# david-gimeno/tailored-avsr

Measured on AMD Instinct MI355X. Metric: utterances/sec fwd+bwd, 12L tailored AV-Branchformer (Conv3d+ResNet-18 lip frontend, fusion, CTC+6L decoder), 4 s clips, batch 32/GPU, higher is better.
Workload: dtype f32

## Files before the change

### tailored-avsr_amd/csrc/gemm.hip

```cpp
#include <algorithm>

#include <cstdlib>
#include "gemm_glds.h"

namespace tavsr {

template <int V>
__global__ __launch_bounds__(256) void splitk_epilogue_kernel(const GemmArgs args) {
  const tavsr_gemm_desc& d = args.d;
  const int64_t mn = (int64_t)d.M * d.N;
  const int nbatch = d.nb1 * d.nb2;
  const int64_t i = ((int64_t)blockIdx.x * 256 + threadIdx.x) * V;
  const int z = blockIdx.y, z1 = z / d.nb2, z2 = z % d.nb2;
  if (d.a_rowsum && z == 0 && i < d.M) {
    const float* rs = d.ws + (int64_t)args.nsplit * nbatch * mn;
    for (int q = 0; q < V && i + q < d.M; ++q) {
      float v = 0.f;
      for (int s = 0; s < args.nsplit; ++s) v += rs[(int64_t)s * d.M + i + q];
      d.a_rowsum[i + q] = d.alpha * v;
    }
  }
  if (i >= mn) return;
  const int m = (int)(i / d.N), n = (int)(i % d.N);
  float v[V];
// ... 154 lines not shown
    __syncthreads();
    int kt0 = 0;
    for (; kt0 + 2 * PF < nk; kt0 += PF) {
#pragma unroll
      for (int u = 0; u < PF; ++u) kstep(kt0 + u, ra[(u + 1) % PF], rb[(u + 1) % PF], true, true, fast_tag);
    }
    for (; kt0 < nk; kt0 += PF) {
#pragma unroll
      for (int u = 0; u < PF; ++u) {
        const int kt = kt0 + u;
        if (kt < nk) kstep(kt, ra[(u + 1) % PF], rb[(u + 1) % PF], kt + 1 < nk, kt + 1 + PF < nk, fast_tag);
      }
    }
  };
  if (fast) run_loop(std::true_type{});
  else run_loop(std::false_type{});

  finish_tile<TM, TN>(d, args.nsplit, acc, asum, want_rowsum, m0, n0, wm, wn, lr, lk, z1, z2, coff, (int)blockIdx.z);
}

__device__ float g_zero_page[16];

template <int ROWS, bool KMAJOR, int NT, bool B_SIDE>
struct TailOperand : PlainOperand<ROWS, KMAJOR, NT, B_SIDE> {
  using P = PlainOperand<ROWS, KMAJOR, NT, B_SIDE>;
  int kofs[P::L::NR];
  __device__ __forceinline__ explicit TailOperand(const TileCtx& c_) : P(c_) {
#pragma unroll
    for (int i = 0; i < P::L::NR; ++i) {
      const int q = i * NT + this->c.tid;
      kofs[i] = KMAJOR ? q / (ROWS / 4) : ((q & 7) ^ (((q >> 3) >> 1) & 7)) * 4;
    }
  }
  __device__ __forceinline__ void issue(int kt, float* img) {
    const TileCtx& c = this->c;
    const int kleft = c.kend - (c.kbeg + kt * kBK);
    const float* g = this->gk + kt * this->kstep;
#pragma unroll
    for (int i = 0; i < P::L::NR; ++i) {
      const float* chunk = g + this->off[i];
      dma16(kofs[i] < kleft ? chunk : g_zero_page, img + (i * NT + c.wave * 64) * 4);
    }
  }
  __device__ __forceinline__ static void zero_past(float* img, int kt_len, int tid) {
    const int k4 = (kt_len + 3) & ~3;
    if (!KMAJOR)
      for (int r = tid; r < ROWS; r += NT)
        for (int kk = kt_len; kk < k4; ++kk) img[r * 32 + ((((kk >> 2) ^ ((r >> 1) & 7))) << 2) + (kk & 3)] = 0.f;
  }
};

template <int BM, int BN, int NT, bool AK, bool BKM>
struct TailSource : SourceDefaults {
  using HA = TailOperand<BM, AK, NT, false>;
  using HB = TailOperand<BN, BKM, NT, true>;
  static constexpr int kDma = HA::kDma + HB::kDma;
  const TileCtx& c;
  HA a;
  HB b;
  __device__ __forceinline__ explicit TailSource(const TileCtx& c_) : c(c_), a(c_), b(c_) {}
  __device__ __forceinline__ int steps() const { return (c.kend - c.kbeg + kBK - 1) / kBK; }
  __device__ __forceinline__ void issue(int kt, float* stage) {
    a.issue(kt, stage);
    b.issue(kt, stage + BM * kBK);
  }
  __device__ __forceinline__ void fix_last(float* stage, int klen, int kt, int tid) const {
    const int kt_len = klen - kt * kBK;
    HA::zero_past(stage, kt_len, tid);
    HB::zero_past(stage + BM * kBK, kt_len, tid);
    __syncthreads();
  }
};
template <int BM, int BN, int NT, bool AK, bool BKM>
struct SourceFor<3, false, BM, BN, NT, AK, BKM> {
  using type = TailSource<BM, BN, NT, AK, BKM>;
};

constexpr int kMaxGroup = 12;
struct GroupArgs {
  tavsr_gemm_desc d[kMaxGroup];
  int tile_start[kMaxGroup + 1];
  int tiles_n[kMaxGroup];
  int n;
  int vec_epi;
};

template <int BM, int BN, int WM, int WN, int S, int MINW, bool AK, bool BKM>
__global__ __launch_bounds__(WM* WN * 64, MINW)
void gemm_glds_grouped_kernel(const GroupArgs g) {
  const int bid = xcd_remap(blockIdx.x, gridDim.x);
  int pi = 0;
#pragma unroll
  for (int i = 1; i < kMaxGroup; ++i)
    if (i < g.n && bid >= g.tile_start[i]) pi = i;
  glds_tile<BM, BN, WM, WN, S, AK, BKM>(g.d[pi], g.d[pi].K, 1, g.tiles_n[pi], bid - g.tile_start[pi], g.vec_epi != 0, 0);
}

// ... 438 lines not shown
```

### tailored-avsr_amd/csrc/gemm_conv.hip

```cpp
#include <algorithm>
#include <vector>

#include "gemm_glds.h"

namespace tavsr {

constexpr int kOrdRuns = 80;
struct TileOrder {
  int nruns;
  int start[kOrdRuns];
  int cum[kOrdRuns + 1];
  int w[kOrdRuns];
};

__host__ __device__ inline void tile_order_map(const TileOrder& o, int b, int tiles_m, int tiles_n, int& mt, int& nt) {
  const int per = 8 * tiles_n;
  const int g = b / per, j = b - g * per, s0 = 8 * g;
  int r0 = 0;
  while (r0 + 1 < o.nruns && o.cum[r0 + 1] <= s0) ++r0;
  bool uniform = s0 + 8 <= tiles_m;
  if (uniform) {
    int r7 = r0;
    while (r7 + 1 < o.nruns && o.cum[r7 + 1] <= s0 + 7) ++r7;
    uniform = o.w[r7] == o.w[r0];
// ... 12 lines not shown
  const unsigned long long taps = (H - 1) * W >= H * (W - 1) ? 0x862053714ull : 0x862071534ull;
  const int tap = (int)((taps >> (4 * rank)) & 15);
  return (rem / tpt) * tiles_n + tap * tpt + rem % tpt;
}

__host__ __device__ inline void dw_xcd_order(int j, int tiles_m, int tiles_n, int ns, int& zs, int& q) {
  const int tiles = tiles_m * tiles_n;
  zs = j / tiles;
  q = j - zs * tiles;
  if (tiles_n % 9 != 0) return;
  const int per = tiles_m * (tiles_n / 9);
  const int rank = j / (ns * per), rem = j - rank * (ns * per);
  zs = rem / per;
  q = rank * per + rem - zs * per;
}

struct ConvGeom {
  int cs, p0, Ho, Wo;
  bool c9;
  __device__ __forceinline__ explicit ConvGeom(const tavsr_gemm_desc& d) {
    cs = d.conv_stride > 1 ? d.conv_stride : 1;
    c9 = d.conv_taps != 1;
    p0 = d.conv_taps == 90 ? 1 : 0;
    Ho = (d.conv_H - 1 - 2 * p0) / cs + 1;
    Wo = (d.conv_W - 1 - 2 * p0) / cs + 1;
  }
};

template <int BM, int NT>
struct ImageRows {
  using L = GLoader<BM, false, NT>;
  int64_t off[L::NR];
  uint32_t mask[L::NR];
  __device__ __forceinline__ void issue(const TileCtx& c, bool c9, int kk, int tap, float* img) const {
    const tavsr_gemm_desc& d = c.d;
    const int toff = c9 ? (tap / 3 - 1) * d.conv_W + (tap % 3 - 1) : 0;
    const int64_t delta = (int64_t)toff * d.conv_C + (kk - tap * d.conv_C);
#pragma unroll
    for (int i = 0; i < L::NR; ++i)
      dma16(((mask[i] >> tap) & 1u) ? c.A + off[i] + delta : d.conv_zero, img + (i * NT + c.wave * 64) * 4);
  }
};

template <int BM, int NT>
struct ConvRowsA {
  using R = ImageRows<BM, NT>;
  static constexpr int kDma = R::L::NR;
  const TileCtx& c;
  bool c9;
  R rows;
  __device__ __forceinline__ explicit ConvRowsA(const TileCtx& c_) : c(c_) {
    const tavsr_gemm_desc& d = c.d;
    const ConvGeom g(d);
    c9 = g.c9;
    R::L::offsets(d.lda, c.m0, d.M, c.tid, rows.off);
#pragma unroll
    for (int i = 0; i < R::L::NR; ++i) {
      const int m = min(c.m0 + ((i * NT + c.tid) >> 3), d.M - 1);
      const int x = (m % g.Wo) * g.cs + g.p0, y = ((m / g.Wo) % g.Ho) * g.cs + g.p0;
      if (g.cs > 1 || g.p0) rows.off[i] += ((int64_t)((m / (g.Wo * g.Ho)) * d.conv_H + y) * d.conv_W + x - m) * d.conv_C;
      uint32_t mk = 0;
#pragma unroll
      for (int tap = 0; tap < 9; ++tap)
        mk |= (uint32_t)((unsigned)(y + tap / 3 - 1) < (unsigned)d.conv_H && (unsigned)(x + tap % 3 - 1) < (unsigned)d.conv_W) << tap;
      rows.mask[i] = g.c9 ? mk : 1u;
    }
  }
  __device__ __forceinline__ void issue(int kt, float* img) {
    const int kk = c.kbeg + kt * kBK;
    rows.issue(c, c9, kk, kk / c.d.conv_C, img);
  }
};
template <int BM, int BN, int NT, bool BKM>
struct SourceFor<1, false, BM, BN, NT, false, BKM> {
  using type = PairSource<ConvRowsA<BM, NT>, PlainOperand<BN, BKM, NT, true>, BM>;
};

template <int BM, int BN, int NT, bool BKM>
struct PosMajorRowsSource : SourceDefaults {
  using R = ImageRows<BM, NT>;
  using LB = GLoader<BN, BKM, NT>;
  static constexpr int kDma = R::L::NR + LB::NR;
  static constexpr bool kPosMajorRows = true;
  const TileCtx& c;
  PosMajor pm{};
  uint32_t taps = 0;
  int tap, cb, nk;
  bool c9;
  R rows;
  int64_t offB[LB::NR];
  __device__ __forceinline__ explicit PosMajorRowsSource(const TileCtx& c_) : c(c_) {
    const tavsr_gemm_desc& d = c.d;
    const ConvGeom g(d);
    c9 = g.c9;
    LB::offsets(d.ldb, c.n0, d.N, c.tid, offB);
    pm.H = g.Ho; pm.W = g.Wo;
    pm.st = g.cs; pm.HI = d.conv_H; pm.WI = d.conv_W;
    pm.n = d.M / (g.Ho * g.Wo);
    const int vlo = c.m0 / pm.n, vhi = min(c.m0 + BM - 1, d.M - 1) / pm.n;
    for (int v = vlo; v <= vhi; ++v) {
      int y, x;
      pm.pos(v, y, x);
      taps |= pm.taps(y, x);
      pm.rp = y * g.Wo + x;
    }
    pm.uni = vlo == vhi;
    pm.base = vlo * pm.n;
    nk = 0;
    for (int t = 0; t < 9; ++t) {
      const int lo = max(c.kbeg, t * d.conv_C), hi = min(c.kend, (t + 1) * d.conv_C);
      if (((taps >> t) & 1u) && hi > lo) nk += (hi - lo) / kBK;
    }
    tap = c.kbeg / d.conv_C;
    cb = (c.kbeg - tap * d.conv_C) / kBK;
    if (!((taps >> tap) & 1u)) {
      const uint32_t up = taps >> (tap + 1) << (tap + 1);
      tap = up ? __builtin_ctz(up) : 9;
      cb = 0;
    }
#pragma unroll
    for (int i = 0; i < R::L::NR; ++i) {
      const int q = i * NT + c.tid, row = q >> 3;
      const int r = min(c.m0 + row, d.M - 1);
      int y, x, img;
      if (pm.uni) {
        y = pm.rp / g.Wo; x = pm.rp - y * g.Wo; img = r - pm.base;
      } else {
        const int v = r / pm.n;
        pm.pos(v, y, x);
        img = r - v * pm.n;
      }
      rows.off[i] = ((int64_t)img * (d.conv_H * d.conv_W) + g.cs * y * d.conv_W + g.cs * x) * d.lda + ((q & 7) ^ ((row >> 1) & 7)) * 4;
      rows.mask[i] = pm.taps(y, x);
    }
  }
  __device__ __forceinline__ int steps() const { return nk; }
  __device__ __forceinline__ const PosMajor* row_map() const { return &pm; }
  __device__ __forceinline__ void issue(int, float* stage) {
    const tavsr_gemm_desc& d = c.d;
    const int ktap = tap, kk = tap * d.conv_C + cb * kBK;
    const int wrap = (cb + 1) * kBK >= d.conv_C;
    const uint32_t up = taps >> (tap + 1) << (tap + 1);
    cb = wrap ? 0 : cb + 1;
    tap = !wrap ? tap : up ? __builtin_ctz(up) : 9;
    rows.issue(c, c9, kk, ktap, stage);
    LB::issue(c.B + (BKM ? (int64_t)kk * d.ldb : kk), offB, stage + BM * kBK, c.wave);
  }
};
template <int BM, int BN, int NT, bool BKM>
struct SourceFor<1, true, BM, BN, NT, false, BKM> {
  using type = PosMajorRowsSource<BM, BN, NT, BKM>;
};

template <int BN, int NT>
struct PatchB {
  using L = GLoader<BN, true, NT>;
  static constexpr int kDma = L::NR;
  const TileCtx& c;
  const ConvGeom g;
  int ox[L::NR], oy[L::NR], img[L::NR];
  int sb, salo, sahi, tapoff, cb, dy, dx;
  __device__ __forceinline__ explicit PatchB(const TileCtx& c_) : c(c_), g(c_.d) {
    const tavsr_gemm_desc& d = c.d;
    const int sa = kBK / g.Wo;
    sb = kBK - sa * g.Wo;
    sahi = sa / g.Ho;
    salo = sa - sahi * g.Ho;
    const int tap = c.n0 / d.conv_C;
    cb = c.n0 - tap * d.conv_C;
    dy = g.c9 ? tap / 3 - 1 : 0;
    dx = g.c9 ? tap % 3 - 1 : 0;
    tapoff = dy * d.conv_W + dx;
#pragma unroll
    for (int i = 0; i < L::NR; ++i) {
      const int m = c.kbeg + (i * NT + c.tid) / (BN / 4);
      const int t = m / g.Wo;
      ox[i] = m - t * g.Wo;
      img[i] = t / g.Ho;
      oy[i] = t - img[i] * g.Ho;
    }
  }
  __device__ __forceinline__ void issue(int, float* dst) {
    const tavsr_gemm_desc& d = c.d;
#pragma unroll
    for (int i = 0; i < L::NR; ++i) {
      const int r = (((i * NT + c.tid) % (BN / 4)) * 4);
      const int x = ox[i] * g.cs + g.p0, y = oy[i] * g.cs + g.p0;
      const bool ok = (unsigned)(y + dy) < (unsigned)d.conv_H && (unsigned)(x + dx) < (unsigned)d.conv_W;
      const int64_t pix = (int64_t)(img[i] * d.conv_H + y) * d.conv_W + x;
      dma16(ok ? c.B + (pix + tapoff) * d.conv_C + cb + r : d.conv_zero, dst + (i * NT + c.wave * 64) * 4);
      int nx = ox[i] + sb;
      const int w1 = nx >= g.Wo ? 1 : 0;
      nx -= w1 ? g.Wo : 0;
      int ny = oy[i] + salo + w1;
      const int w2 = ny >= g.Ho ? 1 : 0;
      ny -= w2 ? g.Ho : 0;
      ox[i] = nx; oy[i] = ny; img[i] += sahi + w2;
    }
  }
};
template <int BM, int BN, int NT>
struct SourceFor<2, false, BM, BN, NT, true, true> {
  using type = PairSource<PlainOperand<BM, true, NT, false>, PatchB<BN, NT>, BM>;
};

template <int BM, int BN, int NT>
struct PatchWalkSource : SourceDefaults {
  using LA = GLoader<BM, true, NT>;
  using LB = GLoader<BN, true, NT>;
  static constexpr int kDma = LA::NR + LB::NR;
  const TileCtx& c;
  const ConvGeom g;
  int64_t offA[LA::NR];
  int tapoff, cb, dy, dx;
  int n, i0, nk;
  int v = 0, img = 0, x = 0, y = 0;
  __device__ __forceinline__ static int rowsum_n0(const tavsr_gemm_desc& d) { return 4 * d.conv_C; }
  __device__ __forceinline__ bool ok(int py, int px) const {
    return (unsigned)(g.cs * py + dy) < (unsigned)c.d.conv_H && (unsigned)(g.cs * px + dx) < (unsigned)c.d.conv_W;
  }
  __device__ __forceinline__ explicit PatchWalkSource(const TileCtx& c_) : c(c_), g(c_.d) {
    const tavsr_gemm_desc& d = c.d;
    const int tap = c.n0 / d.conv_C;
    cb = c.n0 - tap * d.conv_C;
    dy = g.c9 ? tap / 3 - 1 : 0;
    dx = g.c9 ? tap % 3 - 1 : 0;
    tapoff = dy * d.conv_W + dx;
    const int P = g.Ho * g.Wo;
    i0 = c.kbeg / P;
    n = (c.kend - c.kbeg) / P;
    LA::offsets(d.lda, c.m0, d.M, c.tid, offA);
#pragma unroll
    for (int i = 0; i < LA::NR; ++i) offA[i] -= (int64_t)((i * NT + c.tid) / (BM / 4)) * d.lda;
    if (n % kBK == 0) {
      int ny = 0, nx = 0;
      for (int py = 0; py < g.Ho; ++py) ny += (unsigned)(g.cs * py + dy) < (unsigned)d.conv_H;
      for (int px = 0; px < g.Wo; ++px) nx += (unsigned)(g.cs * px + dx) < (unsigned)d.conv_W;
      nk = (n / kBK) * ny * nx;
    } else {
      nk = 0;
      int prev = 0, py = 0, px = 0;
      for (int pv = 0; pv < P; ++pv) {
        if (ok(py, px)) {
          const int s_lo = max(pv * n / kBK, prev), s_hi = ((pv + 1) * n - 1) / kBK + 1;
          if (s_hi > s_lo) { nk += s_hi - s_lo; prev = s_hi; }
        }
        if (++px == g.Wo) { px = 0; ++py; }
      }
    }
  }
  __device__ __forceinline__ int steps() const { return nk; }
  __device__ __forceinline__ void advance() {
    img += kBK;
    while (img >= n) {
      img -= n;
      ++v;
      if (++x == g.Wo) { x = 0; ++y; }
    }
  }
  __device__ __forceinline__ int64_t locate(int kl, int& py, int& px, int& pimg) const {
    int pv = v;
    pimg = img + kl;
    py = y; px = x;
    while (pimg >= n) {
      pimg -= n;
      ++pv;
      if (++px == g.Wo) { px = 0; ++py; }
    }
    pimg += i0;
    return (int64_t)pimg * (g.Ho * g.Wo) + pv;
  }
  __device__ __forceinline__ void issue(int, float* stage) {
    const tavsr_gemm_desc& d = c.d;
    for (;;) {
      bool any = false;
      int end = img + kBK, py = y, px = x;
      for (;;) {
        any |= ok(py, px);
        if (end <= n) break;
        end -= n;
        if (++px == g.Wo) { px = 0; ++py; }
      }
      if (any) break;
      advance();
    }
#pragma unroll
    for (int i = 0; i < LA::NR; ++i) {
      int py, px, pimg;
      const int64_t pix = locate((i * NT + c.tid) / (BM / 4), py, px, pimg);
      dma16(c.A + pix * d.lda + offA[i], stage + (i * NT + c.wave * 64) * 4);
    }
#pragma unroll
    for (int i = 0; i < LB::NR; ++i) {
      const int r = (((i * NT + c.tid) % (BN / 4)) * 4);
      int py, px, pimg;
      locate((i * NT + c.tid) / (BN / 4), py, px, pimg);
      const int64_t pix = ((int64_t)pimg * d.conv_H + g.cs * py) * d.conv_W + g.cs * px;
      dma16(ok(py, px) ? c.B + (pix + tapoff) * d.conv_C + cb + r : d.conv_zero, stage + BM * kBK + (i * NT + c.wave * 64) * 4);
    }
    advance();
  }
};
template <int BM, int BN, int NT>
struct SourceFor<2, true, BM, BN, NT, true, true> {
  using type = PatchWalkSource<BM, BN, NT>;
};

struct StemGeom {
  int T, H, W, Ho, Wo;
  __device__ __forceinline__ explicit StemGeom(const tavsr_gemm_desc& d)
      : T(d.conv_C), H(d.conv_H), W(d.conv_W), Ho((d.conv_H - 1) / 2 + 1), Wo((d.conv_W - 1) / 2 + 1) {}
};

template <int BM, int NT>
struct Stem4A {
  static_assert(NT == 256, "the two-taps-per-thread decoding assumes 8 rows per gather instruction");
  static constexpr int kDma = BM * kBK / NT;
  const TileCtx& c;
  const StemGeom g;
  int base[kDma], mask[kDma];
  int kk0, kk1;
  __device__ __forceinline__ explicit Stem4A(const TileCtx& c_) : c(c_), g(c_.d) {
    const int p = c.tid & 31;
    kk0 = ((((p >> 2) ^ (c.wave & 7))) << 2) + (p & 3);
    kk1 = ((((p >> 2) ^ ((c.wave + 4) & 7))) << 2) + (p & 3);
#pragma unroll
    for (int i = 0; i < kDma; ++i) {
      const int row = i * 8 + (c.tid >> 5);
      const int m = min(c.m0 + row, c.d.M - 1);
      const int wo = m % g.Wo, ho = (m / g.Wo) % g.Ho, ft = m / (g.Wo * g.Ho);
      const int t = ft % g.T, hy = 2 * ho - 3, wx = 2 * wo - 3;
      base[i] = (ft * g.H + hy) * g.W + wx;
      int mk = 0;
#pragma unroll
      for (int q = 0; q < 5; ++q) mk |= (int)((unsigned)(t + q - 2) < (unsigned)g.T) << q;
#pragma unroll
      for (int q = 0; q < 7; ++q)
        mk |= ((int)((unsigned)(hy + q) < (unsigned)g.H) << (8 + q)) | ((int)((unsigned)(wx + q) < (unsigned)g.W) << (16 + q));
      mask[i] = mk;
    }
  }
  __device__ __forceinline__ void issue(int kt, float* img) {
    int tapoff[2], sh[2];
#pragma unroll
    for (int q = 0; q < 2; ++q) {
      const int k = c.kbeg + kt * kBK + (q ? kk1 : kk0);
      const int a = k / 49, r = k - 49 * a, b = r / 7, cc = r - 7 * b;
      tapoff[q] = ((a - 2) * g.H + b) * g.W + cc;
      sh[q] = k < 245 ? (a | ((8 + b) << 8) | ((16 + cc) << 16)) : -1;
    }
#pragma unroll
    for (int i = 0; i < kDma; ++i) {
      const int q = i & 1, mk = mask[i];
      const bool ok = sh[q] >= 0 && (((mk >> (sh[q] & 31)) & (mk >> ((sh[q] >> 8) & 31)) & (mk >> ((sh[q] >> 16) & 31))) & 1);
      dma4(ok ? c.A + (base[i] + tapoff[q]) : c.d.conv_zero, img + i * NT + c.wave * 64);
    }
  }
};
template <int BM, int BN, int NT>
struct SourceFor<4, false, BM, BN, NT, false, false> {
  using type = PairSource<Stem4A<BM, NT>, PlainOperand<BN, false, NT, true>, BM>;
};

template <int BN, int NT>
struct Stem5B {
  static_assert(BN == 64 && NT == 256, "one k row per wave instruction");
  static constexpr int kDma = BN * kBK / NT;
  const TileCtx& c;
  const StemGeom g;
  int wo, ho, t, off, tapoff, c3, a, b;
  bool nok;
  bool th;
  __device__ __forceinline__ bool frame_row_ok() const {
    return nok && (unsigned)(t + a - 2) < (unsigned)g.T && (unsigned)(2 * ho - 3 + b) < (unsigned)g.H;
  }
  __device__ __forceinline__ explicit Stem5B(const TileCtx& c_) : c(c_), g(c_.d) {
    const int nn = c.n0 + (c.tid & 63);
    a = nn / 49; b = (nn % 49) / 7;
    const int cc = nn % 7;
    c3 = cc - 3;
    nok = nn < 245;
    tapoff = ((a - 2) * g.H + b - 3) * g.W + cc - 3;
    const int m = c.kbeg + c.wave;
    wo = m % g.Wo; ho = (m / g.Wo) % g.Ho;
    const int ft = m / (g.Wo * g.Ho);
    t = ft % g.T;
    off = (ft * g.H + 2 * ho) * g.W + 2 * wo;
    th = frame_row_ok();
  }
  __device__ __forceinline__ void issue(int, float* img) {
#pragma unroll
    for (int i = 0; i < kDma; ++i) {
      const bool ok = th && (unsigned)(2 * wo + c3) < (unsigned)g.W;
      dma4(ok ? c.B + (off + tapoff) : c.d.conv_zero, img + i * NT + c.wave * 64);
      wo += 4;
      off += 8;
      if (wo >= g.Wo) {
        wo -= g.Wo;
        off += g.W;
        if (++ho == g.Ho) {
          ho = 0;
          if (++t == g.T) t = 0;
        }
        th = frame_row_ok();
      }
    }
  }
};
template <int BM, int BN, int NT>
struct SourceFor<5, false, BM, BN, NT, true, true> {
  using type = PairSource<PlainOperand<BM, true, NT, false>, Stem5B<BN, NT>, BM>;
};

struct PaddedStemGeom {
  int Hp, Wp, Tp, Ho, Wo, T;
  __device__ __forceinline__ explicit PaddedStemGeom(const tavsr_gemm_desc& d)
      : Hp(d.conv_H), Wp(d.conv_W), Tp(d.conv_C), Ho((d.conv_H - 6) / 2), Wo((d.conv_W - 8) / 2), T(d.conv_C - 5) {}
  __device__ __forceinline__ int pixel(int m) const {
    const int wo = m % Wo, ho = (m / Wo) % Ho, ft = m / (Wo * Ho);
    return (((ft / T) * Tp + ft % T) * Hp + 2 * ho) * Wp + 2 * wo;
  }
};

template <int BM, int NT>
struct Stem6A {
  using L = GLoader<BM, false, NT>;
  static constexpr int kDma = L::NR;
  const TileCtx& c;
  const PaddedStemGeom g;
  int base[L::NR], cl[L::NR];
  __device__ __forceinline__ explicit Stem6A(const TileCtx& c_) : c(c_), g(c_.d) {
#pragma unroll
    for (int i = 0; i < L::NR; ++i) {
      const int q = i * NT + c.tid, row = q >> 3;
      cl[i] = (q & 7) ^ ((row >> 1) & 7);
      base[i] = g.pixel(min(c.m0 + row, c.d.M - 1));
    }
  }
  __device__ __forceinline__ void issue(int kt, float* img) {
#pragma unroll
    for (int i = 0; i < L::NR; ++i) {
      const int ch = (c.kbeg >> 2) + kt * 8 + cl[i], r = ch >> 1, a = r / 7, b = r - 7 * a;
      dma16(c.A + (base[i] + (a * g.Hp + b) * g.Wp + 4 * (ch & 1)), img + (i * NT + c.wave * 64) * 4);
    }
  }
};
template <int BM, int BN, int NT>
struct SourceFor<6, false, BM, BN, NT, false, false> {
  using type = PairSource<Stem6A<BM, NT>, PlainOperand<BN, false, NT, true>, BM>;
};

template <int BN, int NT>
struct Stem7B {
  using L = GLoader<BN, true, NT>;
  static constexpr int kDma = L::NR;
  const TileCtx& c;
  const PaddedStemGeom g;
  int wo[L::NR], ho[L::NR], t[L::NR], off[L::NR];
  int tapoff;
  __device__ __forceinline__ explicit Stem7B(const TileCtx& c_) : c(c_), g(c_.d) {
    constexpr int CPR = BN / 4;
    int ch = (c.n0 >> 2) + (c.tid % CPR);
    if (ch >= 72) ch = 0;
    const int r = ch >> 1, a = r / 7, b = r - 7 * a;
    tapoff = (a * g.Hp + b) * g.Wp + 4 * (ch & 1);
#pragma unroll
    for (int i = 0; i < L::NR; ++i) {
      const int m = c.kbeg + (i * NT + c.tid) / CPR;
      wo[i] = m % g.Wo; ho[i] = (m / g.Wo) % g.Ho; t[i] = (m / (g.Wo * g.Ho)) % g.T;
      off[i] = g.pixel(m);
    }
  }
  __device__ __forceinline__ void issue(int, float* img) {
    constexpr int STEP = 32;
#pragma unroll
    for (int i = 0; i < L::NR; ++i) {
      dma16(c.B + (off[i] + tapoff), img + (i * NT + c.wave * 64) * 4);
      wo[i] += STEP;
      off[i] += 2 * STEP;
      while (wo[i] >= g.Wo) {
        wo[i] -= g.Wo;
        off[i] += 2 * g.Wp - 2 * g.Wo;
        if (++ho[i] == g.Ho) {
          ho[i] = 0;
          off[i] += (g.Hp - 2 * g.Ho) * g.Wp;
          if (++t[i] == g.T) { t[i] = 0; off[i] += (g.Tp - g.T) * g.Hp * g.Wp; }
        }
      }
    }
  }
};
template <int BM, int BN, int NT>
struct SourceFor<7, false, BM, BN, NT, true, true> {
  using type = PairSource<PlainOperand<BM, true, NT, false>, Stem7B<BN, NT>, BM>;
};

struct GemmArgsOrd {
  GemmArgs g;
  TileOrder ord;
};
template <int CONV, bool PM>
struct TileMap<CONV, PM, true> {
  __device__ __forceinline__ static const GemmArgs& map(const GemmArgsOrd& x, int& bid, int& zidx) {
    bid = xcd_remap(blockIdx.x, gridDim.x);
    zidx = blockIdx.z;
    if (x.ord.nruns > 0) {
      int mt, nt;
      tile_order_map(x.ord, blockIdx.x, x.g.tiles_m, x.g.tiles_n, mt, nt);
      bid = mt * x.g.tiles_n + nt;
    }
    return x.g;
  }
  __device__ __forceinline__ static const GemmArgs& map(const GemmArgs& args, int& bid, int& zidx) {
    bid = xcd_remap(blockIdx.x, gridDim.x);
    zidx = blockIdx.z;
    if (args.zmap) {
      const int tiles = gridDim.x, l = blockIdx.x + tiles * blockIdx.z, j = l >> 3;
      int zs = j / tiles;
      bid = j % tiles;
      if constexpr (PM && CONV == 2) {
// ... 197 lines not shown
```

### tailored-avsr_amd/csrc/gemm_glds.h

```cpp
#pragma once
#include <type_traits>

#include "common.h"

namespace tavsr {

typedef float f32x16 __attribute__((ext_vector_type(16)));
constexpr int kBK = 32;

struct GemmArgs {
  tavsr_gemm_desc d;
  int kchunk;
  int nsplit;
  int tiles_m, tiles_n;
  int vec_epi;
  int zmap;
  int n_big, kunit;
};

template <int ROWS, int BK, bool KMAJOR>
struct Tile {
  static constexpr int LD = KMAJOR ? (ROWS + 4) : (BK + 4);
  static constexpr int SIZE = KMAJOR ? BK * LD : ROWS * LD;
};
// ... 280 lines not shown
  }
}

static bool aligned16(const void* p) { return (reinterpret_cast<uintptr_t>(p) & 15) == 0; }
static bool vec_epi_ok(const tavsr_gemm_desc& d) {
  return d.N % 4 == 0 && d.ldc % 4 == 0 && d.sC1 % 4 == 0 && d.sC2 % 4 == 0 && aligned16(d.C) && (!d.bias || aligned16(d.bias)) &&
         (!d.Z || aligned16(d.Z)) && (!d.DZ || aligned16(d.DZ)) &&
         (!d.R || (aligned16(d.R) && d.ldr % 4 == 0 && d.sR1 % 4 == 0 && d.sR2 % 4 == 0)) && (!d.ws || aligned16(d.ws));
}

typedef __attribute__((address_space(3))) float lds_float;
typedef const __attribute__((address_space(1))) float glb_float;

template <int ROWS, bool KMAJOR, int NT>
struct GLoader {
  static constexpr int NR = ROWS * 8 / NT;
  static_assert(ROWS * 8 % NT == 0, "tile must divide over the block");
  __device__ static __forceinline__ void offsets(int64_t ld, int row0, int nrows, int tid, int64_t (&off)[NR]) {
#pragma unroll
    for (int i = 0; i < NR; ++i) {
      const int q = i * NT + tid;
      if (KMAJOR) {
        const int k = q / (ROWS / 4);
        int r = row0 + (q % (ROWS / 4)) * 4;
        if (r + 3 >= nrows) r = row0;
        off[i] = (int64_t)k * ld + r;
      } else {
        const int row = q >> 3, cp = q & 7;
        const int cl = cp ^ ((row >> 1) & 7);
        off[i] = (int64_t)min(row0 + row, nrows - 1) * ld + cl * 4;
      }
    }
  }
  __device__ static __forceinline__ void issue(const float* __restrict__ g, const int64_t (&off)[NR],
                                               float* __restrict__ stage, int wave) {
#pragma unroll
    for (int i = 0; i < NR; ++i)
      __builtin_amdgcn_global_load_lds((glb_float*)(g + off[i]), (lds_float*)(stage + (i * NT + wave * 64) * 4), 16, 0, 0);
  }
};

__device__ __forceinline__ void dma16(const float* src, float* dst) {
  __builtin_amdgcn_global_load_lds((glb_float*)src, (lds_float*)dst, 16, 0, 0);
}
__device__ __forceinline__ void dma4(const float* src, float* dst) {
  __builtin_amdgcn_global_load_lds((glb_float*)src, (lds_float*)dst, 4, 0, 0);
}

#ifndef TAVSR_GEMM_SB
#define TAVSR_GEMM_SB 1
#endif
#if TAVSR_GEMM_SB
#define GEMM_SB() __builtin_amdgcn_sched_barrier(0)
#else
#define GEMM_SB()
#endif

template <int ROWS, bool KMAJOR>
__device__ __forceinline__ void read_frag_g(const float* __restrict__ s, int row, int g, int lk, float (&f)[4]) {
  if (KMAJOR) {
    const float* p = s + (g * 8 + 4 * lk) * ROWS + row;
#pragma unroll
    for (int j = 0; j < 4; ++j) f[j] = p[j * ROWS];
  } else {
    const float4 v = *reinterpret_cast<const float4*>(s + row * 32 + (((2 * g + lk) ^ ((row >> 1) & 7)) << 2));
    f[0] = v.x; f[1] = v.y; f[2] = v.z; f[3] = v.w;
  }
}

template <int N>
__device__ __forceinline__ void wait_vmcnt() {
  asm volatile("s_waitcnt vmcnt(%0)" ::"n"(N) : "memory");
}

#ifdef TAVSR_GEMM_TRACE
constexpr int kTraceMax = 1 << 15;
static __device__ unsigned long long g_trace[kTraceMax][6];
static __device__ unsigned int g_trace_n;
#define TAVSR_TRACE_DECL unsigned long long tr_t[4], tr_c[4]; tr_t[0] = wall_clock64(); tr_t[1] = tr_t[0]; tr_c[1] = tr_c[2] = 0;
#define TAVSR_TRACE_AT(i) { tr_t[i] = wall_clock64(); tr_c[i] = __builtin_readcyclecounter(); }
static int trace_read_unit(unsigned long long* out, int max_rows) {
  unsigned int n = 0;
  if (hipDeviceSynchronize() != hipSuccess) return -1;
  if (hipMemcpyFromSymbol(&n, HIP_SYMBOL(g_trace_n), sizeof(n)) != hipSuccess) return -1;
  int rows = (int)(n < (unsigned)kTraceMax ? n : kTraceMax);
  if (rows > max_rows) rows = max_rows;
  if (rows > 0 && hipMemcpyFromSymbol(out, HIP_SYMBOL(g_trace), (size_t)rows * 6 * sizeof(unsigned long long)) != hipSuccess) return -1;
  n = 0;
// ... 6 lines not shown
#define TAVSR_TRACE_AT(i)
#endif

struct TileCtx {
  const tavsr_gemm_desc& d;
  const float* A;
  const float* B;
  int m0, n0;
  int kbeg, kend;
  int tid, wave;
};

struct SourceDefaults {
  static constexpr bool kPosMajorRows = false;
  __device__ __forceinline__ const PosMajor* row_map() const { return nullptr; }
  __device__ __forceinline__ static int rowsum_n0(const tavsr_gemm_desc&) { return 0; }
  __device__ __forceinline__ void fix_last(float*, int, int, int) const {}
};

template <int ROWS, bool KMAJOR, int NT, bool B_SIDE>
struct PlainOperand {
  using L = GLoader<ROWS, KMAJOR, NT>;
  static constexpr int kDma = L::NR;
  const TileCtx& c;
  int64_t off[L::NR];
  const float* gk;
  int64_t kstep;
  __device__ __forceinline__ explicit PlainOperand(const TileCtx& c_) : c(c_) {
    const int64_t ld = B_SIDE ? c.d.ldb : c.d.lda;
    L::offsets(ld, B_SIDE ? c.n0 : c.m0, B_SIDE ? c.d.N : c.d.M, c.tid, off);
    kstep = KMAJOR ? (int64_t)kBK * ld : kBK;
    gk = (B_SIDE ? c.B : c.A) + (KMAJOR ? (int64_t)c.kbeg * ld : c.kbeg);
  }
  __device__ __forceinline__ void issue(int kt, float* img) { L::issue(gk + kt * kstep, off, img, c.wave); }
};

template <class HA, class HB, int BM>
struct PairSource : SourceDefaults {
  static constexpr int kDma = HA::kDma + HB::kDma;
  HA a;
  HB b;
  int nk;
  __device__ __forceinline__ explicit PairSource(const TileCtx& c) : a(c), b(c), nk((c.kend - c.kbeg) / kBK) {}
  __device__ __forceinline__ int steps() const { return nk; }
  __device__ __forceinline__ void issue(int kt, float* stage) {
    a.issue(kt, stage);
    b.issue(kt, stage + BM * kBK);
  }
};

template <int CONV, bool PM, int BM, int BN, int NT, bool AK, bool BKM>
struct SourceFor;
template <int BM, int BN, int NT, bool AK, bool BKM>
struct SourceFor<0, false, BM, BN, NT, AK, BKM> {
  using type = PairSource<PlainOperand<BM, AK, NT, false>, PlainOperand<BN, BKM, NT, true>, BM>;
};

template <int BM, int BN, int WM, int WN, int S, bool AK, bool BKM, int KW = 1, int CONV = 0, bool PM = false>
__device__ __forceinline__ void glds_tile(const tavsr_gemm_desc& d, int kchunk, int nsplit, int tiles_n, int bid, bool vec_epi,
                                          int zidx, int n_big = 0, int kunit = 0) {
  constexpr int BK = kBK, NG = BK / 8;
  static_assert(NG % KW == 0, "k-groups must divide over the wave sets");
  static_assert(!PM || KW == 1, "position-major order: one wave set");
  constexpr int NT = WM * WN * KW * 64;
  constexpr int TM = BM / WM / 32, TN = BN / WN / 32;
  using Src = typename SourceFor<CONV, PM, BM, BN, NT, AK, BKM>::type;
  constexpr int ASZ = BM * BK, STAGE = (BM + BN) * BK;
  constexpr int G = Src::kDma;
  static_assert((S - 2) * G <= 63, "vmcnt field");
  __shared__ __attribute__((aligned(1024))) float smem[S * STAGE];

  const int tid = threadIdx.x;
  const int lane = tid & 63;
  const int wave = __builtin_amdgcn_readfirstlane(tid >> 6);
  const int kw = wave / (WM * WN), w2 = wave % (WM * WN);
  const int wm = w2 / WN, wn = w2 % WN;
  const int lr = lane & 31, lk = lane >> 5;

  TAVSR_TRACE_DECL
  const int m0 = (bid / tiles_n) * BM;
  const int n0 = (bid % tiles_n) * BN;
  const int z1 = blockIdx.y / d.nb2, z2 = blockIdx.y % d.nb2;
  const float* A = d.A + z1 * d.sA1 + z2 * d.sA2;
  const float* B = d.B + z1 * d.sB1 + z2 * d.sB2;
  const int64_t coff = z1 * d.sC1 + z2 * d.sC2;

  f32x16 acc[TM][TN];
#pragma unroll
  for (int i = 0; i < TM; ++i)
#pragma unroll
    for (int j = 0; j < TN; ++j)
#pragma unroll
      for (int r = 0; r < 16; ++r) acc[i][j][r] = 0.f;
  float asum[TM];
#pragma unroll
  for (int i = 0; i < TM; ++i) asum[i] = 0.f;
  float bpre[TN];
#pragma unroll
  for (int j = 0; j < TN; ++j) {
    const int n = n0 + wn * TN * 32 + j * 32 + lr;
    bpre[j] = (d.bias && nsplit == 1 && n < d.N) ? d.bias[n] : 0.f;
  }

  const int kbeg = zidx * kchunk + min(zidx, n_big) * kunit;
  const int kend = min(d.K, kbeg + kchunk + (zidx < n_big ? kunit : 0));
  const TileCtx ctx{d, A, B, m0, n0, kbeg, kend, tid, wave};
  Src src(ctx);
  const int nk = src.steps();
  const bool want_rowsum = d.a_rowsum != nullptr && n0 == Src::rowsum_n0(d) && wn == 0;

  const int arow = wm * TM * 32 + lr, brow = wn * TN * 32 + lr;
  auto compute = [&](int st) {
    const float* a_s = smem + st * STAGE;
    const float* b_s = a_s + ASZ;
    float af[2][TM][4], bf[2][TN][4];
#pragma unroll
    for (int i = 0; i < TM; ++i) read_frag_g<BM, AK>(a_s, arow + i * 32, kw, lk, af[0][i]);
#pragma unroll
    for (int j = 0; j < TN; ++j) read_frag_g<BN, BKM>(b_s, brow + j * 32, kw, lk, bf[0][j]);
#pragma unroll
    for (int q = 0; q < NG / KW; ++q) {
      const int c = q & 1;
      if (q + 1 < NG / KW) {
#pragma unroll
        for (int i = 0; i < TM; ++i) read_frag_g<BM, AK>(a_s, arow + i * 32, kw + (q + 1) * KW, lk, af[c ^ 1][i]);
#pragma unroll
        for (int j = 0; j < TN; ++j) read_frag_g<BN, BKM>(b_s, brow + j * 32, kw + (q + 1) * KW, lk, bf[c ^ 1][j]);
      }
      GEMM_SB();
#pragma unroll
      for (int kk = 0; kk < 4; ++kk)
#pragma unroll
        for (int i = 0; i < TM; ++i)
#pragma unroll
          for (int j = 0; j < TN; ++j)
            acc[i][j] = __builtin_amdgcn_mfma_f32_32x32x2f32(af[c][i][kk], bf[c][j][kk], acc[i][j], 0, 0, 0);
#pragma unroll
      for (int i = 0; i < TM; ++i) asum[i] += (af[c][i][0] + af[c][i][1]) + (af[c][i][2] + af[c][i][3]);
      GEMM_SB();
    }
  };

#pragma unroll
  for (int j = 0; j < S - 1; ++j)
    if (j < nk) src.issue(j, smem + j * STAGE);
  int st = 0;
  int kt = 0;
  for (; kt + S - 1 < nk; ++kt) {
    wait_vmcnt<(S - 2) * G>();
    __builtin_amdgcn_s_barrier();
#ifdef TAVSR_GEMM_TRACE
    if (kt == 0) TAVSR_TRACE_AT(1)
#endif
    const int sn = st == 0 ? S - 1 : st - 1;
    src.issue(kt + S - 1, smem + sn * STAGE);
    compute(st);
    st = st + 1 == S ? 0 : st + 1;
  }
  for (; kt < nk; ++kt) {
    wait_vmcnt<0>();
    __builtin_amdgcn_s_barrier();
    if (kt == nk - 1 && ((kend - kbeg) & 3) != 0) src.fix_last(smem + st * STAGE, kend - kbeg, kt, tid);
    compute(st);
    st = st + 1 == S ? 0 : st + 1;
  }
  TAVSR_TRACE_AT(2)
  if (KW > 1) {
    constexpr int PER = TM * TN * 16;
    float* red = smem;
    float* rsum = smem + (KW - 1) * WM * WN * PER * 64;
    static_assert(((KW - 1) * WM * WN * (PER + TM) * 64) <= S * STAGE, "reduction must fit in the staging ring");
    __syncthreads();
    if (kw > 0) {
      float* r0 = red + ((kw - 1) * WM * WN + w2) * PER * 64 + lane;
#pragma unroll
      for (int i = 0; i < TM; ++i)
#pragma unroll
        for (int j = 0; j < TN; ++j)
#pragma unroll
          for (int r = 0; r < 16; ++r) r0[((i * TN + j) * 16 + r) * 64] = acc[i][j][r];
#pragma unroll
      for (int i = 0; i < TM; ++i) rsum[(((kw - 1) * WM * WN + w2) * TM + i) * 64 + lane] = asum[i];
    }
    __syncthreads();
    if (kw > 0) return;
#pragma unroll
    for (int s2 = 0; s2 < KW - 1; ++s2) {
      const float* r0 = red + (s2 * WM * WN + w2) * PER * 64 + lane;
#pragma unroll
      for (int i = 0; i < TM; ++i)
#pragma unroll
        for (int j = 0; j < TN; ++j)
#pragma unroll
          for (int r = 0; r < 16; ++r) acc[i][j][r] += r0[((i * TN + j) * 16 + r) * 64];
#pragma unroll
      for (int i = 0; i < TM; ++i) asum[i] += rsum[((s2 * WM * WN + w2) * TM + i) * 64 + lane];
// ... 81 lines not shown
```

Before: 412.4.

## Interleave per-piece global-to-LDS DMA issues between MFMAs in GEMM main loop

Splits each source's bulk issue() into per-piece issue_piece() calls and, in the steady-state K loop, slots each DMA issue behind successive MFMA instructions using scheduling barriers and asm register constraints. The aim is to spread the global_load_lds issue cost across the matrix-core stream instead of front-loading it before compute, hiding address-generation and issue latency. Conv sources 4 and 5 keep the DMA-first order, and stateful sources are restructured so their advance logic runs on piece 0, including a changed initial img state. This adds scheduling complexity and risks changing register pressure or the order of the stateful iterator updates.

New measurement: 413.5 (median of 2 runs). About the same (+0.3%).

```diff
diff --git a/tailored-avsr_amd/csrc/gemm.hip b/tailored-avsr_amd/csrc/gemm.hip
--- a/tailored-avsr_amd/csrc/gemm.hip
+++ b/tailored-avsr_amd/csrc/gemm.hip
@@ -210,15 +210,11 @@
       kofs[i] = KMAJOR ? q / (ROWS / 4) : ((q & 7) ^ (((q >> 3) >> 1) & 7)) * 4;
     }
   }
-  __device__ __forceinline__ void issue(int kt, float* img) {
+  __device__ __forceinline__ void issue_piece(int kt, float* img, int i) {
     const TileCtx& c = this->c;
     const int kleft = c.kend - (c.kbeg + kt * kBK);
-    const float* g = this->gk + kt * this->kstep;
-#pragma unroll
-    for (int i = 0; i < P::L::NR; ++i) {
-      const float* chunk = g + this->off[i];
-      dma16(kofs[i] < kleft ? chunk : g_zero_page, img + (i * NT + c.wave * 64) * 4);
-    }
+    const float* chunk = this->gk + kt * this->kstep + this->off[i];
+    dma16(kofs[i] < kleft ? chunk : g_zero_page, P::L::dst(img, i, c.wave));
   }
   __device__ __forceinline__ static void zero_past(float* img, int kt_len, int tid) {
     const int k4 = (kt_len + 3) & ~3;
@@ -238,9 +234,9 @@
   HB b;
   __device__ __forceinline__ explicit TailSource(const TileCtx& c_) : c(c_), a(c_), b(c_) {}
   __device__ __forceinline__ int steps() const { return (c.kend - c.kbeg + kBK - 1) / kBK; }
-  __device__ __forceinline__ void issue(int kt, float* stage) {
-    a.issue(kt, stage);
-    b.issue(kt, stage + BM * kBK);
+  __device__ __forceinline__ void issue_piece(int kt, float* stage, int i) {
+    if (i < HA::kDma) a.issue_piece(kt, stage, i);
+    else b.issue_piece(kt, stage + BM * kBK, i - HA::kDma);
   }
   __device__ __forceinline__ void fix_last(float* stage, int klen, int kt, int tid) const {
     const int kt_len = klen - kt * kBK;
diff --git a/tailored-avsr_amd/csrc/gemm_conv.hip b/tailored-avsr_amd/csrc/gemm_conv.hip
--- a/tailored-avsr_amd/csrc/gemm_conv.hip
+++ b/tailored-avsr_amd/csrc/gemm_conv.hip
@@ -68,13 +68,11 @@
   using L = GLoader<BM, false, NT>;
   int64_t off[L::NR];
   uint32_t mask[L::NR];
-  __device__ __forceinline__ void issue(const TileCtx& c, bool c9, int kk, int tap, float* img) const {
+  __device__ __forceinline__ void issue_piece(const TileCtx& c, bool c9, int kk, int tap, float* img, int i) const {
     const tavsr_gemm_desc& d = c.d;
     const int toff = c9 ? (tap / 3 - 1) * d.conv_W + (tap % 3 - 1) : 0;
     const int64_t delta = (int64_t)toff * d.conv_C + (kk - tap * d.conv_C);
-#pragma unroll
-    for (int i = 0; i < L::NR; ++i)
-      dma16(((mask[i] >> tap) & 1u) ? c.A + off[i] + delta : d.conv_zero, img + (i * NT + c.wave * 64) * 4);
+    dma16(((mask[i] >> tap) & 1u) ? c.A + off[i] + delta : d.conv_zero, L::dst(img, i, c.wave));
   }
 };
 
@@ -102,9 +100,9 @@
       rows.mask[i] = g.c9 ? mk : 1u;
     }
   }
-  __device__ __forceinline__ void issue(int kt, float* img) {
+  __device__ __forceinline__ void issue_piece(int kt, float* img, int i) {
     const int kk = c.kbeg + kt * kBK;
-    rows.issue(c, c9, kk, kk / c.d.conv_C, img);
+    rows.issue_piece(c, c9, kk, kk / c.d.conv_C, img, i);
   }
 };
 template <int BM, int BN, int NT, bool BKM>
@@ -122,6 +120,7 @@
   PosMajor pm{};
   uint32_t taps = 0;
   int tap, cb, nk;
+  int ktap = 0, kk = 0;
   bool c9;
   R rows;
   int64_t offB[LB::NR];
@@ -172,15 +171,22 @@
   }
   __device__ __forceinline__ int steps() const { return nk; }
   __device__ __forceinline__ const PosMajor* row_map() const { return &pm; }
-  __device__ __forceinline__ void issue(int, float* stage) {
+  __device__ __forceinline__ void issue_piece(int, float* stage, int i) {
     const tavsr_gemm_desc& d = c.d;
-    const int ktap = tap, kk = tap * d.conv_C + cb * kBK;
-    const int wrap = (cb + 1) * kBK >= d.conv_C;
-    const uint32_t up = taps >> (tap + 1) << (tap + 1);
-    cb = wrap ? 0 : cb + 1;
-    tap = !wrap ? tap : up ? __builtin_ctz(up) : 9;
-    rows.issue(c, c9, kk, ktap, stage);
-    LB::issue(c.B + (BKM ? (int64_t)kk * d.ldb : kk), offB, stage + BM * kBK, c.wave);
+    if (i == 0) {
+      ktap = tap;
+      kk = tap * d.conv_C + cb * kBK;
+      const int wrap = (cb + 1) * kBK >= d.conv_C;
+      const uint32_t up = taps >> (tap + 1) << (tap + 1);
+      cb = wrap ? 0 : cb + 1;
+      tap = !wrap ? tap : up ? __builtin_ctz(up) : 9;
+    }
+    if (i < R::L::NR) {
+      rows.issue_piece(c, c9, kk, ktap, stage, i);
+    } else {
+      const int j = i - R::L::NR;
+      dma16(c.B + (BKM ? (int64_t)kk * d.ldb : kk) + offB[j], LB::dst(stage + BM * kBK, j, c.wave));
+    }
   }
 };
 template <int BM, int BN, int NT, bool BKM>
@@ -216,23 +222,20 @@
       oy[i] = t - img[i] * g.Ho;
     }
   }
-  __device__ __forceinline__ void issue(int, float* dst) {
+  __device__ __forceinline__ void issue_piece(int, float* dst, int i) {
     const tavsr_gemm_desc& d = c.d;
-#pragma unroll
-    for (int i = 0; i < L::NR; ++i) {
-      const int r = (((i * NT + c.tid) % (BN / 4)) * 4);
-      const int x = ox[i] * g.cs + g.p0, y = oy[i] * g.cs + g.p0;
-      const bool ok = (unsigned)(y + dy) < (unsigned)d.conv_H && (unsigned)(x + dx) < (unsigned)d.conv_W;
-      const int64_t pix = (int64_t)(img[i] * d.conv_H + y) * d.conv_W + x;
-      dma16(ok ? c.B + (pix + tapoff) * d.conv_C + cb + r : d.conv_zero, dst + (i * NT + c.wave * 64) * 4);
-      int nx = ox[i] + sb;
-      const int w1 = nx >= g.Wo ? 1 : 0;
-      nx -= w1 ? g.Wo : 0;
-      int ny = oy[i] + salo + w1;
-      const int w2 = ny >= g.Ho ? 1 : 0;
-      ny -= w2 ? g.Ho : 0;
-      ox[i] = nx; oy[i] = ny; img[i] += sahi + w2;
-    }
+    const int r = (((i * NT + c.tid) % (BN / 4)) * 4);
+    const int x = ox[i] * g.cs + g.p0, y = oy[i] * g.cs + g.p0;
+    const bool ok = (unsigned)(y + dy) < (unsigned)d.conv_H && (unsigned)(x + dx) < (unsigned)d.conv_W;
+    const int64_t pix = (int64_t)(img[i] * d.conv_H + y) * d.conv_W + x;
+    dma16(ok ? c.B + (pix + tapoff) * d.conv_C + cb + r : d.conv_zero, L::dst(dst, i, c.wave));
+    int nx = ox[i] + sb;
+    const int w1 = nx >= g.Wo ? 1 : 0;
+    nx -= w1 ? g.Wo : 0;
+    int ny = oy[i] + salo + w1;
+    const int w2 = ny >= g.Ho ? 1 : 0;
+    ny -= w2 ? g.Ho : 0;
+    ox[i] = nx; oy[i] = ny; img[i] += sahi + w2;
   }
 };
 template <int BM, int BN, int NT>
@@ -250,7 +253,7 @@
   int64_t offA[LA::NR];
   int tapoff, cb, dy, dx;
   int n, i0, nk;
-  int v = 0, img = 0, x = 0, y = 0;
+  int v = 0, img = -kBK, x = 0, y = 0;
   __device__ __forceinline__ static int rowsum_n0(const tavsr_gemm_desc& d) { return 4 * d.conv_C; }
   __device__ __forceinline__ bool ok(int py, int px) const {
     return (unsigned)(g.cs * py + dy) < (unsigned)c.d.conv_H && (unsigned)(g.cs * px + dx) < (unsigned)c.d.conv_W;
@@ -306,35 +309,34 @@
     pimg += i0;
     return (int64_t)pimg * (g.Ho * g.Wo) + pv;
   }
-  __device__ __forceinline__ void issue(int, float* stage) {
+  __device__ __forceinline__ void issue_piece(int, float* stage, int i) {
     const tavsr_gemm_desc& d = c.d;
-    for (;;) {
-      bool any = false;
-      int end = img + kBK, py = y, px = x;
+    if (i == 0) {
+      advance();
       for (;;) {
-        any |= ok(py, px);
-        if (end <= n) break;
-        end -= n;
-        if (++px == g.Wo) { px = 0; ++py; }
-      }
-      if (any) break;
-      advance();
-    }
-#pragma unroll
-    for (int i = 0; i < LA::NR; ++i) {
-      int py, px, pimg;
+        bool any = false;
+        int end = img + kBK, py = y, px = x;
+        for (;;) {
+          any |= ok(py, px);
+          if (end <= n) break;
+          end -= n;
+          if (++px == g.Wo) { px = 0; ++py; }
+        }
+        if (any) break;
+        advance();
+      }
+    }
+    int py, px, pimg;
+    if (i < LA::NR) {
       const int64_t pix = locate((i * NT + c.tid) / (BM / 4), py, px, pimg);
-      dma16(c.A + pix * d.lda + offA[i], stage + (i * NT + c.wave * 64) * 4);
-    }
-#pragma unroll
-    for (int i = 0; i < LB::NR; ++i) {
-      const int r = (((i * NT + c.tid) % (BN / 4)) * 4);
-      int py, px, pimg;
-      locate((i * NT + c.tid) / (BN / 4), py, px, pimg);
+      dma16(c.A + pix * d.lda + offA[i], LA::dst(stage, i, c.wave));
+    } else {
+      const int j = i - LA::NR;
+      const int r = (((j * NT + c.tid) % (BN / 4)) * 4);
+      locate((j * NT + c.tid) / (BN / 4), py, px, pimg);
       const int64_t pix = ((int64_t)pimg * d.conv_H + g.cs * py) * d.conv_W + g.cs * px;
-      dma16(ok(py, px) ? c.B + (pix + tapoff) * d.conv_C + cb + r : d.conv_zero, stage + BM * kBK + (i * NT + c.wave * 64) * 4);
-    }
-    advance();
+      dma16(ok(py, px) ? c.B + (pix + tapoff) * d.conv_C + cb + r : d.conv_zero, LB::dst(stage + BM * kBK, j, c.wave));
+    }
   }
 };
 template <int BM, int BN, int NT>
@@ -376,21 +378,14 @@
       mask[i] = mk;
     }
   }
-  __device__ __forceinline__ void issue(int kt, float* img) {
-    int tapoff[2], sh[2];
-#pragma unroll
-    for (int q = 0; q < 2; ++q) {
-      const int k = c.kbeg + kt * kBK + (q ? kk1 : kk0);
-      const int a = k / 49, r = k - 49 * a, b = r / 7, cc = r - 7 * b;
-      tapoff[q] = ((a - 2) * g.H + b) * g.W + cc;
-      sh[q] = k < 245 ? (a | ((8 + b) << 8) | ((16 + cc) << 16)) : -1;
-    }
-#pragma unroll
-    for (int i = 0; i < kDma; ++i) {
-      const int q = i & 1, mk = mask[i];
-      const bool ok = sh[q] >= 0 && (((mk >> (sh[q] & 31)) & (mk >> ((sh[q] >> 8) & 31)) & (mk >> ((sh[q] >> 16) & 31))) & 1);
-      dma4(ok ? c.A + (base[i] + tapoff[q]) : c.d.conv_zero, img + i * NT + c.wave * 64);
-    }
+  __device__ __forceinline__ void issue_piece(int kt, float* img, int i) {
+    const int k = c.kbeg + kt * kBK + ((i & 1) ? kk1 : kk0);
+    const int a = k / 49, r = k - 49 * a, b = r / 7, cc = r - 7 * b;
+    const int tapoff = ((a - 2) * g.H + b) * g.W + cc;
+    const int sh = k < 245 ? (a | ((8 + b) << 8) | ((16 + cc) << 16)) : -1;
+    const int mk = mask[i];
+    const bool ok = sh >= 0 && (((mk >> (sh & 31)) & (mk >> ((sh >> 8) & 31)) & (mk >> ((sh >> 16) & 31))) & 1);
+    dma4(ok ? c.A + (base[i] + tapoff) : c.d.conv_zero, img + i * NT + c.wave * 64);
   }
 };
 template <int BM, int BN, int NT>
@@ -424,22 +419,19 @@
     off = (ft * g.H + 2 * ho) * g.W + 2 * wo;
     th = frame_row_ok();
   }
-  __device__ __forceinline__ void issue(int, float* img) {
-#pragma unroll
-    for (int i = 0; i < kDma; ++i) {
-      const bool ok = th && (unsigned)(2 * wo + c3) < (unsigned)g.W;
-      dma4(ok ? c.B + (off + tapoff) : c.d.conv_zero, img + i * NT + c.wave * 64);
-      wo += 4;
-      off += 8;
-      if (wo >= g.Wo) {
-        wo -= g.Wo;
-        off += g.W;
-        if (++ho == g.Ho) {
-          ho = 0;
-          if (++t == g.T) t = 0;
-        }
-        th = frame_row_ok();
-      }
+  __device__ __forceinline__ void issue_piece(int, float* img, int i) {
+    const bool ok = th && (unsigned)(2 * wo + c3) < (unsigned)g.W;
+    dma4(ok ? c.B + (off + tapoff) : c.d.conv_zero, img + i * NT + c.wave * 64);
+    wo += 4;
+    off += 8;
+    if (wo >= g.Wo) {
+      wo -= g.Wo;
+      off += g.W;
+      if (++ho == g.Ho) {
+        ho = 0;
+        if (++t == g.T) t = 0;
+      }
+      th = frame_row_ok();
     }
   }
 };
@@ -473,12 +465,9 @@
       base[i] = g.pixel(min(c.m0 + row, c.d.M - 1));
     }
   }
-  __device__ __forceinline__ void issue(int kt, float* img) {
-#pragma unroll
-    for (int i = 0; i < L::NR; ++i) {
-      const int ch = (c.kbeg >> 2) + kt * 8 + cl[i], r = ch >> 1, a = r / 7, b = r - 7 * a;
-      dma16(c.A + (base[i] + (a * g.Hp + b) * g.Wp + 4 * (ch & 1)), img + (i * NT + c.wave * 64) * 4);
-    }
+  __device__ __forceinline__ void issue_piece(int kt, float* img, int i) {
+    const int ch = (c.kbeg >> 2) + kt * 8 + cl[i], r = ch >> 1, a = r / 7, b = r - 7 * a;
+    dma16(c.A + (base[i] + (a * g.Hp + b) * g.Wp + 4 * (ch & 1)), L::dst(img, i, c.wave));
   }
 };
 template <int BM, int BN, int NT>
@@ -507,21 +496,18 @@
       off[i] = g.pixel(m);
     }
   }
-  __device__ __forceinline__ void issue(int, float* img) {
+  __device__ __forceinline__ void issue_piece(int, float* img, int i) {
     constexpr int STEP = 32;
-#pragma unroll
-    for (int i = 0; i < L::NR; ++i) {
-      dma16(c.B + (off[i] + tapoff), img + (i * NT + c.wave * 64) * 4);
-      wo[i] += STEP;
-      off[i] += 2 * STEP;
-      while (wo[i] >= g.Wo) {
-        wo[i] -= g.Wo;
-        off[i] += 2 * g.Wp - 2 * g.Wo;
-        if (++ho[i] == g.Ho) {
-          ho[i] = 0;
-          off[i] += (g.Hp - 2 * g.Ho) * g.Wp;
-          if (++t[i] == g.T) { t[i] = 0; off[i] += (g.Tp - g.T) * g.Hp * g.Wp; }
-        }
+    dma16(c.B + (off[i] + tapoff), L::dst(img, i, c.wave));
+    wo[i] += STEP;
+    off[i] += 2 * STEP;
+    while (wo[i] >= g.Wo) {
+      wo[i] -= g.Wo;
+      off[i] += 2 * g.Wp - 2 * g.Wo;
+      if (++ho[i] == g.Ho) {
+        ho[i] = 0;
+        off[i] += (g.Hp - 2 * g.Ho) * g.Wp;
+        if (++t[i] == g.T) { t[i] = 0; off[i] += (g.Tp - g.T) * g.Hp * g.Wp; }
       }
     }
   }
diff --git a/tailored-avsr_amd/csrc/gemm_glds.h b/tailored-avsr_amd/csrc/gemm_glds.h
--- a/tailored-avsr_amd/csrc/gemm_glds.h
+++ b/tailored-avsr_amd/csrc/gemm_glds.h
@@ -336,12 +336,7 @@
       }
     }
   }
-  __device__ static __forceinline__ void issue(const float* __restrict__ g, const int64_t (&off)[NR],
-                                               float* __restrict__ stage, int wave) {
-#pragma unroll
-    for (int i = 0; i < NR; ++i)
-      __builtin_amdgcn_global_load_lds((glb_float*)(g + off[i]), (lds_float*)(stage + (i * NT + wave * 64) * 4), 16, 0, 0);
-  }
+  __device__ static __forceinline__ float* dst(float* __restrict__ img, int i, int wave) { return img + (i * NT + wave * 64) * 4; }
 };
 
 __device__ __forceinline__ void dma16(const float* src, float* dst) {
@@ -358,6 +353,16 @@
 #define GEMM_SB() __builtin_amdgcn_sched_barrier(0)
 #else
 #define GEMM_SB()
+#endif
+#if TAVSR_GEMM_SB && defined(__HIP_DEVICE_COMPILE__)
+#define GEMM_ISSUED(x) asm volatile("" ::"v"(x))
+#define GEMM_HELD(x) asm volatile("" : "+v"(x))
+#else
+#define GEMM_ISSUED(x)
+#define GEMM_HELD(x)
+#endif
+#ifndef TAVSR_GEMM_DMA_FIRST
+#define TAVSR_GEMM_DMA_FIRST 0
 #endif
 
 template <int ROWS, bool KMAJOR>
@@ -430,7 +435,7 @@
     kstep = KMAJOR ? (int64_t)kBK * ld : kBK;
     gk = (B_SIDE ? c.B : c.A) + (KMAJOR ? (int64_t)c.kbeg * ld : c.kbeg);
   }
-  __device__ __forceinline__ void issue(int kt, float* img) { L::issue(gk + kt * kstep, off, img, c.wave); }
+  __device__ __forceinline__ void issue_piece(int kt, float* img, int i) { dma16(gk + kt * kstep + off[i], L::dst(img, i, c.wave)); }
 };
 
 template <class HA, class HB, int BM>
@@ -441,9 +446,9 @@
   int nk;
   __device__ __forceinline__ explicit PairSource(const TileCtx& c) : a(c), b(c), nk((c.kend - c.kbeg) / kBK) {}
   __device__ __forceinline__ int steps() const { return nk; }
-  __device__ __forceinline__ void issue(int kt, float* stage) {
-    a.issue(kt, stage);
-    b.issue(kt, stage + BM * kBK);
+  __device__ __forceinline__ void issue_piece(int kt, float* stage, int i) {
+    if (i < HA::kDma) a.issue_piece(kt, stage, i);
+    else b.issue_piece(kt, stage + BM * kBK, i - HA::kDma);
   }
 };
 
@@ -466,6 +471,8 @@
   constexpr int ASZ = BM * BK, STAGE = (BM + BN) * BK;
   constexpr int G = Src::kDma;
   static_assert((S - 2) * G <= 63, "vmcnt field");
+  static_assert(G < (NG / KW) * 4 * TM * TN, "a K-step's pieces go behind its MFMAs 1 .. G");
+  constexpr bool kDmaFirst = TAVSR_GEMM_DMA_FIRST || CONV == 4 || CONV == 5;
   __shared__ __attribute__((aligned(1024))) float smem[S * STAGE];
 
   const int tid = threadIdx.x;
@@ -508,7 +515,11 @@
   const bool want_rowsum = d.a_rowsum != nullptr && n0 == Src::rowsum_n0(d) && wn == 0;
 
   const int arow = wm * TM * 32 + lr, brow = wn * TN * 32 + lr;
-  auto compute = [&](int st) {
+  auto issue_step = [&](int kn, float* sn) {
+#pragma unroll
+    for (int i = 0; i < G; ++i) src.issue_piece(kn, sn, i);
+  };
+  auto compute = [&](int st, auto dma, int kn, float* sn) {
     const float* a_s = smem + st * STAGE;
     const float* b_s = a_s + ASZ;
     float af[2][TM][4], bf[2][TN][4];
@@ -531,8 +542,18 @@
 #pragma unroll
         for (int i = 0; i < TM; ++i)
 #pragma unroll
-          for (int j = 0; j < TN; ++j)
+          for (int j = 0; j < TN; ++j) {
             acc[i][j] = __builtin_amdgcn_mfma_f32_32x32x2f32(af[c][i][kk], bf[c][j][kk], acc[i][j], 0, 0, 0);
+            constexpr int PER = TM * TN, NM = (NG / KW) * 4 * PER;
+            const int n = ((q * 4 + kk) * TM + i) * TN + j;
+            if (decltype(dma)::value && n >= 1 && n <= G) {
+              GEMM_ISSUED(acc[i][j]);
+              GEMM_SB();
+              src.issue_piece(kn, sn, n - 1);
+              if (n + 1 < NM) GEMM_HELD(af[((n + 1) / (4 * PER)) & 1][((n + 1) / TN) % TM][((n + 1) / PER) % 4]);
+              GEMM_SB();
+            }
+          }
 #pragma unroll
       for (int i = 0; i < TM; ++i) asum[i] += (af[c][i][0] + af[c][i][1]) + (af[c][i][2] + af[c][i][3]);
       GEMM_SB();
@@ -541,7 +562,7 @@
 
 #pragma unroll
   for (int j = 0; j < S - 1; ++j)
-    if (j < nk) src.issue(j, smem + j * STAGE);
+    if (j < nk) issue_step(j, smem + j * STAGE);
   int st = 0;
   int kt = 0;
   for (; kt + S - 1 < nk; ++kt) {
@@ -551,15 +572,19 @@
     if (kt == 0) TAVSR_TRACE_AT(1)
 #endif
     const int sn = st == 0 ? S - 1 : st - 1;
-    src.issue(kt + S - 1, smem + sn * STAGE);
-    compute(st);
+    if constexpr (kDmaFirst) {
+      issue_step(kt + S - 1, smem + sn * STAGE);
+      compute(st, std::false_type{}, 0, nullptr);
+    } else {
+      compute(st, std::true_type{}, kt + S - 1, smem + sn * STAGE);
+    }
     st = st + 1 == S ? 0 : st + 1;
   }
   for (; kt < nk; ++kt) {
     wait_vmcnt<0>();
     __builtin_amdgcn_s_barrier();
     if (kt == nk - 1 && ((kend - kbeg) & 3) != 0) src.fix_last(smem + st * STAGE, kend - kbeg, kt, tid);
-    compute(st);
+    compute(st, std::false_type{}, 0, nullptr);
     st = st + 1 == S ? 0 : st + 1;
   }
   TAVSR_TRACE_AT(2)
```
